# ateme-developers/SVT-AV1-1

Hardware: AMD Instinct MI355X
Metric: 64x64 SAD-search blocks/sec (higher is better)
Workload: dtype u8; 1 GPU; configs[1]: 64x64 full-pel SAD hierarchical ME (centre check + HME L0/L1/L2 + 64x64-area full-pel search of 85 square PUs), 1080p 8-bit, one reference list

## Files before the change

svt-av1-1_amd/csrc/me_hme_impl.h:

```cpp
#pragma once


typedef const __attribute__((address_space(1))) uint32_t gmem_u32;
struct __attribute__((packed, aligned(1))) gmem_u32x4 { uint32_t v[4]; };

__device__ __forceinline__ uint32_t ldu32(const uint8_t* p)
{
    const uintptr_t a = reinterpret_cast<uintptr_t>(p);
    gmem_u32* q = (gmem_u32*)(a & ~(uintptr_t)3);
    const uint32_t sh = (uint32_t)(a & 3u);
    const uint32_t lo = q[0];
    const uint32_t hi = sh ? q[1] : 0u;
    return __builtin_amdgcn_alignbyte(hi, lo, sh);
}

__device__ __forceinline__ uint32_t ldu32_nb(const uint8_t* p)
{
    const uintptr_t a = reinterpret_cast<uintptr_t>(p);
    gmem_u32* q = (gmem_u32*)(a & ~(uintptr_t)3);
    return __builtin_amdgcn_alignbyte(q[1], q[0], (uint32_t)(a & 3u));
}

__device__ __forceinline__ uint32_t wave_sum_u32(uint32_t v)
{
#pragma unroll
    for (int m = 1; m < 64; m <<= 1) v += __shfl_xor(v, m);
    return v;
}

#ifdef SVTHIP_HME_NO_PRIO
#define HME_PRIO(p) do { } while (0)
#else
#define HME_PRIO(p) __builtin_amdgcn_s_setprio(p)
#endif
#ifdef SVTHIP_HME_STAMPS
__device__ unsigned long long g_hme_stamps[8192 * 4 * 8];
#define HME_STAMP(i)                                                                                                          \
    do {                                                                                                                      \
        if (lane == 0 && sbi < 8192u) g_hme_stamps[((size_t)sbi * 4 + (threadIdx.x >> 6)) * 8 + (i)] = __builtin_amdgcn_s_memtime(); \
    } while (0)
__device__ unsigned long long g_hme_loop_phase[2 * 4];
#define HME_LOOP_T(var) const unsigned long long var = __builtin_amdgcn_s_memtime()
#define HME_LOOP_ADD(slot, t1, t0)                                                                                \
    do {                                                                                                          \
        if (lane == 0) atomicAdd(&g_hme_loop_phase[(W == 64 ? 4 : 0) + (slot)], (unsigned long long)((t1) - (t0))); \
    } while (0)
#else
#define HME_STAMP(i) do { } while (0)
#define HME_LOOP_T(var) do { } while (0)
#define HME_LOOP_ADD(slot, t1, t0) do { } while (0)
#endif

constexpr int kHmeLdsPerWave = 7 * 1024;

__device__ __forceinline__ void load_ref_block64(const uint8_t* ref, uint32_t ref_stride, int lane, uint32_t (&tv)[8])
{
    const uint32_t c = (uint32_t)lane & 15u, r0 = (uint32_t)lane >> 4;
    const uint8_t* rp = ref + (size_t)r0 * ref_stride + 4u * c;
#pragma unroll
    for (int k = 0; k < 8; k++) tv[k] = ldu32_nb(rp + (size_t)(4 * k) * ref_stride);
}

__device__ __forceinline__ uint32_t sad_ref_block64(const uint32_t (&tv)[8], const uint32_t* src_lds, int lane)
{
    const uint32_t c = (uint32_t)lane & 15u, r0 = (uint32_t)lane >> 4;
    uint32_t acc4 = 0;
#pragma unroll
    for (int k = 0; k < 8; k++) acc4 = __builtin_amdgcn_sad_u8(src_lds[(r0 + 4 * k) * 16 + c], tv[k], acc4);
    return wave_sum_u32(acc4);
}

__device__ uint32_t wave_block_sad(const uint8_t* src, uint32_t src_stride, const uint8_t* ref, uint32_t ref_stride,
                                   uint32_t H, uint32_t W, int lane, const uint32_t* src_lds = nullptr)
{
    if (src_lds && W == 64 && H == 32) {
        uint32_t tv[8];
        load_ref_block64(ref, ref_stride, lane, tv);
        return sad_ref_block64(tv, src_lds, lane);
    }
    if (W == 64 && (H & 3u) == 0) {
        const uint32_t c = (uint32_t)lane & 15u, r0 = (uint32_t)lane >> 4;
        const uint8_t* sp = src + (size_t)r0 * src_stride + 4u * c;
        const uint8_t* rp = ref + (size_t)r0 * ref_stride + 4u * c;
        uint32_t acc4 = 0;
        for (uint32_t r = 0; r < H; r += 16) {
            uint32_t sv[4], tv[4];
#pragma unroll
            for (int k = 0; k < 4; k++) {
                const bool in = r + 4u * (uint32_t)k < H;
                sv[k] = in ? *reinterpret_cast<const uint32_t*>(sp + (size_t)(4 * k) * src_stride) : 0u;
                tv[k] = in ? ldu32_nb(rp + (size_t)(4 * k) * ref_stride) : 0u;
            }
#pragma unroll
            for (int k = 0; k < 4; k++) acc4 = __builtin_amdgcn_sad_u8(sv[k], tv[k], acc4);
            sp += (size_t)16 * src_stride;
            rp += (size_t)16 * ref_stride;
        }
        return wave_sum_u32(acc4);
    }
    const uint32_t ndw = (W + 3) >> 2;
    const uint32_t n = H * ndw;
    uint32_t acc = 0;
    for (uint32_t i = lane; i < n; i += 64) {
        const uint32_t r = i / ndw, c = i - r * ndw;
        uint32_t s = ldu32(src + (size_t)r * src_stride + 4 * c);
        uint32_t t = ldu32(ref + (size_t)r * ref_stride + 4 * c);
        const uint32_t rem = W - 4 * c;
        if (rem < 4) {
            const uint32_t m = (1u << (8 * rem)) - 1u;
            s &= m;
            t &= m;
        }
        acc = __builtin_amdgcn_sad_u8(s, t, acc);
    }
    return wave_sum_u32(acc);
}

__device__ void wave_sad_loop_generic(const uint8_t* src, uint32_t src_stride, const uint8_t* ref, uint32_t ref_stride,
                                      uint32_t H, uint32_t W, uint32_t ref_stride_raw, int sw, int sh, int lane,
                                      uint32_t* best_sad, int* bx, int* by)
{
    const int npos = sw * sh;
    unsigned long long best = ~0ull;
    const uint32_t ndw = (W + 3) >> 2;
    const uint32_t tail = W & 3u;
    const uint32_t tailmask = tail ? ((1u << (8 * tail)) - 1u) : 0xffffffffu;
#pragma unroll 1
    for (int pos = lane; pos < npos; pos += 64) {
        const int y = pos / sw, x = pos - y * sw;
        const uint8_t* r0 = ref + (size_t)y * ref_stride_raw + x;
        uint32_t acc = 0;
#pragma unroll 1
        for (uint32_t r = 0; r < H; r++) {
            const uint8_t* sp = src + (size_t)r * src_stride;
            const uint8_t* rp = r0 + (size_t)r * ref_stride;
#pragma unroll 2
            for (uint32_t c = 0; c < ndw; c++) {
                uint32_t s = ldu32(sp + 4 * c);
                uint32_t t = ldu32(rp + 4 * c);
                if (c == ndw - 1) {
                    s &= tailmask;
                    t &= tailmask;
                }
                acc = __builtin_amdgcn_sad_u8(s, t, acc);
            }
        }
        const unsigned long long key = ((unsigned long long)acc << 32) | (uint32_t)pos;
        best = key < best ? key : best;
    }
    best = wave_min_u64(best);
    const uint32_t pos = (uint32_t)__builtin_amdgcn_readfirstlane((int)(uint32_t)best);
    *best_sad = (uint32_t)__builtin_amdgcn_readfirstlane((int)(uint32_t)(best >> 32));
    *by = (int)(pos / (uint32_t)sw);
    *bx = (int)(pos - (uint32_t)(*by) * (uint32_t)sw);
}

__device__ __forceinline__ void stage_window_rows(const uint8_t* base, uint32_t ref_stride_raw, int wrows, int pitch, uint32_t* win,
                                                  int lane)
{
    constexpr int NP = 6;
    const int lpr = (pitch + 3) >> 2;
    const int rpp = lpr < 64 ? 64 / lpr : 1;
    const int g = (int)(((uint32_t)lane * ((1u << 16) / (uint32_t)lpr + 1u)) >> 16), q4 = 4 * (lane - g * lpr);
    const bool lane_ok = g < rpp;
    const uintptr_t a0 = reinterpret_cast<uintptr_t>(base) + 4u * (uint32_t)q4;
    for (int r0 = g; r0 < wrows; r0 += NP * rpp) {
        gmem_u32x4 w[NP];
#pragma unroll
        for (int u = 0; u < NP; u++) {
            const int r = min(r0 + u * rpp, wrows - 1);
            const __attribute__((address_space(1))) gmem_u32x4* q = (const __attribute__((address_space(1))) gmem_u32x4*)(a0 + (size_t)r * ref_stride_raw);
#pragma unroll
            for (int k = 0; k < 4; k++) w[u].v[k] = q->v[k];
        }
#pragma unroll
        for (int u = 0; u < NP; u++) {
            const int r = r0 + u * rpp;
            if (lane_ok && r < wrows) {
                uint32_t* o = win + r * pitch + q4;
#pragma unroll
                for (int k = 0; k < 4; k++)
                    if (q4 + k < pitch) o[k] = w[u].v[k];
            }
        }
    }
}

template <int W, bool KEY32 = false>
__device__ void wave_sad_loop_lds(const uint8_t* src, uint32_t src_stride, const uint8_t* ref, uint32_t ref_stride_raw,
                                  int H, int sw, int sh, int lane, uint8_t* lds, int lds_bytes, uint32_t* best_sad,
                                  int* bx, int* by, const uint32_t* shared_src = nullptr)
{
    constexpr int WD = W / 4;
    constexpr int FLUSH = (W == 16) ? 16 : (W == 32 ? 8 : 4);
    const int own_src = shared_src ? 0 : H * WD;
    const uint32_t* srcbuf = shared_src ? shared_src : reinterpret_cast<const uint32_t*>(lds);
    const int noct = (sw + 7) >> 3;
    const int pitch = 2 * noct + WD + 1;
    uint32_t* win = reinterpret_cast<uint32_t*>(lds) + own_src;
    const int avail_rows = (lds_bytes / 4 - own_src) / pitch;
    int band = avail_rows - (2 * H - 2);
    if (band > sh) band = sh;
    if (band < 1) {
        wave_sad_loop_generic(src, src_stride, ref, ref_stride_raw * 2, (uint32_t)H, (uint32_t)W, ref_stride_raw, sw, sh, lane,
                              best_sad, bx, by);
        return;
    }

    for (int i0 = 0; !shared_src && i0 < H * WD; i0 += 256) {
        uint32_t v[4];
#pragma unroll
        for (int k = 0; k < 4; k++) {
            const int i = min(i0 + k * 64 + lane, H * WD - 1);
            const int r = i / WD, c = i - r * WD;
            v[k] = ldu32_nb(src + (uint32_t)r * src_stride + 4u * (uint32_t)c);
        }
#pragma unroll
        for (int k = 0; k < 4; k++) reinterpret_cast<uint32_t*>(lds)[min(i0 + k * 64 + lane, H * WD - 1)] = v[k];
    }

    const int items_row = noct;
    unsigned long long best = ~0ull;
    uint32_t best32 = 0xffffffffu;

    for (int y0 = 0; y0 < sh; y0 += band) {
        const int bh = min(band, sh - y0);
        const int wrows = bh + 2 * H - 2;
        HME_LOOP_T(t_a);
        HME_PRIO(3);
        stage_window_rows(ref + (size_t)y0 * ref_stride_raw, ref_stride_raw, wrows, pitch, win, lane);
        __builtin_amdgcn_wave_barrier();
        asm volatile("s_waitcnt vmcnt(0) lgkmcnt(0)" ::: "memory");
        HME_PRIO(0);
        HME_LOOP_T(t_b);
        HME_LOOP_ADD(0, t_b, t_a);

        const int nitems = items_row * bh;
        int RP = 1, rp_shift = 0;
        while (RP < 8 && nitems * RP * 2 <= 64 && RP * 2 <= H) { RP <<= 1; rp_shift++; }
        const int ipw = 64 >> rp_shift;
        const int part = lane & (RP - 1);
        const uint32_t inv_items = (1u << 20) / (uint32_t)items_row + 1u;
        for (int it0 = 0; it0 < nitems; it0 += ipw) {
            const int item = it0 + (lane >> rp_shift);
            const bool valid = item < nitems;
            const int iy = valid ? (int)(((uint32_t)item * inv_items) >> 20) : 0;
            const int io = valid ? item - iy * items_row : 0;
            uint32_t sad[8];
#pragma unroll
            for (int j = 0; j < 8; j++) sad[j] = 0;
            uint64_t acc0 = 0, acc1 = 0;
            int since = 0;
            for (int r = part; r < H; r += RP) {
                const uint32_t* wr = win + (iy + 2 * r) * pitch + 2 * io;
                const uint32_t* sr = srcbuf + r * WD;
                uint32_t d[WD + 2];
#pragma unroll
                for (int c = 0; c < WD + 2; c++) d[c] = wr[c];
#pragma unroll
                for (int c = 0; c < WD; c++) {
                    const uint32_t sv = sr[c];
                    acc0 = __builtin_amdgcn_qsad_pk_u16_u8(pack64(d[c], d[c + 1]), sv, acc0);
                    acc1 = __builtin_amdgcn_qsad_pk_u16_u8(pack64(d[c + 1], d[c + 2]), sv, acc1);
                }
                if (++since == FLUSH) {
                    since = 0;
                    sad[0] += (uint32_t)acc0 & 0xffffu; sad[1] += ((uint32_t)acc0) >> 16;
                    sad[2] += (uint32_t)(acc0 >> 32) & 0xffffu; sad[3] += (uint32_t)(acc0 >> 48);
                    sad[4] += (uint32_t)acc1 & 0xffffu; sad[5] += ((uint32_t)acc1) >> 16;
                    sad[6] += (uint32_t)(acc1 >> 32) & 0xffffu; sad[7] += (uint32_t)(acc1 >> 48);
                    acc0 = acc1 = 0;
                }
            }
            sad[0] += (uint32_t)acc0 & 0xffffu; sad[1] += ((uint32_t)acc0) >> 16;
            sad[2] += (uint32_t)(acc0 >> 32) & 0xffffu; sad[3] += (uint32_t)(acc0 >> 48);
            sad[4] += (uint32_t)acc1 & 0xffffu; sad[5] += ((uint32_t)acc1) >> 16;
            sad[6] += (uint32_t)(acc1 >> 32) & 0xffffu; sad[7] += (uint32_t)(acc1 >> 48);
            for (int m = 1; m < RP; m <<= 1) {
#pragma unroll
                for (int j = 0; j < 8; j++) sad[j] += __shfl_xor(sad[j], m);
            }
            if (valid && part == 0) {
                const int ys = y0 + iy;
#pragma unroll
                for (int j = 0; j < 8; j++) {
                    const int xs = 8 * io + j;
                    if (xs < sw) {
                        if (KEY32) {
                            best32 = min(best32, (sad[j] << 12) | (uint32_t)(ys * sw + xs));
                        } else {
                            const unsigned long long key = ((unsigned long long)sad[j] << 32) | (uint32_t)(ys * sw + xs);
                            best = key < best ? key : best;
                        }
                    }
                }
            }
        }
        __builtin_amdgcn_wave_barrier();
        HME_LOOP_T(t_c);
        HME_LOOP_ADD(1, t_c, t_b);
    }
    HME_LOOP_T(t_d);
    if (KEY32) {
#pragma unroll
        for (int m = 1; m < 64; m <<= 1) best32 = min(best32, (uint32_t)__shfl_xor((int)best32, m));
        best = ((unsigned long long)(best32 >> 12) << 32) | (best32 & 0xfffu);
    } else {
        best = wave_min_u64(best);
    }
    const uint32_t pos = (uint32_t)__builtin_amdgcn_readfirstlane((int)(uint32_t)best);
    *best_sad = (uint32_t)__builtin_amdgcn_readfirstlane((int)(uint32_t)(best >> 32));
    *by = (int)(pos / (uint32_t)sw);
    *bx = (int)(pos - (uint32_t)(*by) * (uint32_t)sw);
    HME_LOOP_T(t_e);
    HME_LOOP_ADD(2, t_e, t_d);
    HME_LOOP_ADD(3, 1ull, 0ull);
}

template <int W, int H, int SW, int SH>
__device__ void wave_sad_loop_fixed(const uint8_t* ref, uint32_t ref_stride_raw, int lane, uint8_t* lds, const uint32_t* srcbuf,
                                    uint32_t* best_sad, int* bx, int* by)
{
    constexpr int WD = W / 4;
    constexpr int NQ = SW / 4;
    constexpr int RP = 64 / SH;
    constexpr int ROWS = H / RP;
    constexpr int ND = WD + NQ;
    constexpr int PITCH = (ND + 3) & ~3;
    constexpr int WROWS = SH + 2 * H - 2;
    static_assert(RP * SH == 64 && ROWS * RP == H && (RP & (RP - 1)) == 0 && RP >= 2 && RP <= 8, "one wave pass, RP a power of two");
    static_assert(ROWS * W * 255 < 65536 && H * W * 255 < (1 << 20) && SW * SH <= 4096 && (SW & (SW - 1)) == 0, "u16 sums, 32-bit keys");
    static_assert(WROWS * PITCH * 4 <= kHmeLdsPerWave, "the window fits the slice");
    typedef __attribute__((address_space(3))) uint32_t lds_u32;
    typedef uint32_t u32x4_t __attribute__((ext_vector_type(4)));
    typedef uint32_t u32x2_t __attribute__((ext_vector_type(2)));

    uint32_t* win = reinterpret_cast<uint32_t*>(lds);
    HME_PRIO(3);
    stage_window_rows(ref, ref_stride_raw, WROWS, PITCH, win, lane);
    __builtin_amdgcn_wave_barrier();
    asm volatile("s_waitcnt vmcnt(0) lgkmcnt(0)" ::: "memory");
    HME_PRIO(0);

    const int iy = lane / RP, part = lane & (RP - 1);
    const uint32_t* w0 = win + (iy + 2 * part) * PITCH;
    uint64_t acc[NQ];
#pragma unroll
    for (int g = 0; g < NQ; g++) acc[g] = 0;
#pragma unroll
    for (int i = 0; i < ROWS; i++) {
        const int r = part + RP * i;
        const uint32_t* wr = w0 + 2 * RP * i * PITCH;
        lds_u32* wo = (lds_u32*)wr;
        asm("" : "+v"(wo));
        uint32_t d[PITCH];
#pragma unroll
        for (int k = 0; k < PITCH / 4; k++) {
            if (4 * k + 2 >= ND) {
                u32x2_t v = *reinterpret_cast<const u32x2_t*>(wr + 4 * k);
                asm("" : "+v"(v));
                d[4 * k] = v.x; d[4 * k + 1] = v.y; d[4 * k + 2] = d[4 * k + 3] = 0;
            } else {
                u32x4_t v = *reinterpret_cast<const u32x4_t*>(wr + 4 * k);
                asm("" : "+v"(v));
                d[4 * k] = v.x; d[4 * k + 1] = v.y; d[4 * k + 2] = v.z; d[4 * k + 3] = v.w;
            }
        }
        uint64_t odd[ND / 2];
#pragma unroll
        for (int k = 1; k + 1 < ND; k += 2) odd[k / 2] = pack64(wo[k], wo[k + 1]);
        uint32_t sv[WD];
#pragma unroll
        for (int k = 0; k < WD / 4; k++) {
            const uint4 v = *reinterpret_cast<const uint4*>(srcbuf + r * WD + 4 * k);
            sv[4 * k] = v.x; sv[4 * k + 1] = v.y; sv[4 * k + 2] = v.z; sv[4 * k + 3] = v.w;
        }
#pragma unroll
        for (int c = 0; c < WD; c++)
#pragma unroll
            for (int g = 0; g < NQ; g++) {
                const int k = c + g;
                acc[g] = __builtin_amdgcn_qsad_pk_u16_u8((k & 1) ? odd[k / 2] : pack64(d[k], d[k + 1]), sv[c], acc[g]);
            }
    }
    __builtin_amdgcn_wave_barrier();

    uint32_t key = 0xffffffffu;
#pragma unroll
    for (int g = 0; g < NQ; g++) {
        uint32_t v[4] = {(uint32_t)acc[g] & 0xffffu, (uint32_t)acc[g] >> 16, (uint32_t)(acc[g] >> 32) & 0xffffu, (uint32_t)(acc[g] >> 48)};
#pragma unroll
        for (int j = 0; j < 4; j++) {
            v[j] += dpp_fetch<0xB1>(v[j]);
            v[j] += dpp_fetch<0x4E>(v[j]);
            if (RP == 8) v[j] += dpp_fetch<0x141>(v[j]);
        }
        key = min3u((v[0] << 12) | (uint32_t)(4 * g), (v[1] << 12) | (uint32_t)(4 * g + 1), key);
        key = min3u((v[2] << 12) | (uint32_t)(4 * g + 2), (v[3] << 12) | (uint32_t)(4 * g + 3), key);
    }
    key |= (uint32_t)(iy * SW);
    key = min(key, dpp_fetch<0xB1>(key));
    key = min(key, dpp_fetch<0x4E>(key));
    key = min(key, dpp_fetch<0x124>(key));
    key = min(key, dpp_fetch<0x128>(key));
    const uint32_t best = min(min((uint32_t)__builtin_amdgcn_readlane((int)key, 0), (uint32_t)__builtin_amdgcn_readlane((int)key, 16)),
                              min((uint32_t)__builtin_amdgcn_readlane((int)key, 32), (uint32_t)__builtin_amdgcn_readlane((int)key, 48)));
    const uint32_t pos = best & 0xfffu;
    *best_sad = best >> 12;
    *by = (int)(pos / (uint32_t)SW);
    *bx = (int)(pos % (uint32_t)SW);
}

__device__ void wave_sad_loop_l0(const uint8_t* src, uint32_t src_stride, const uint8_t* ref, uint32_t ref_stride_raw, int sw, int sh,
                                 int lane, uint8_t* lds, int lds_bytes, uint32_t* best_sad, int* bx, int* by,
                                 const uint32_t* shared_src = nullptr)
{
    constexpr int H = 8, WD = 4;
    const int own_src = shared_src ? 0 : H * WD;
    const uint32_t* srcbuf = shared_src ? shared_src : reinterpret_cast<const uint32_t*>(lds);
    const int nit = (sw + 15) >> 4;
    const int pitch = 4 * nit + 4;
    uint32_t* win = reinterpret_cast<uint32_t*>(lds) + own_src;
    const int avail_rows = (lds_bytes / 4 - own_src) / pitch;
    int band = avail_rows - (2 * H - 2);
    if (band > sh) band = sh;
    if (band < 1 || sw * sh > 65536) {
        wave_sad_loop_lds<16>(src, src_stride, ref, ref_stride_raw, H, sw, sh, lane, lds, lds_bytes, best_sad, bx, by, shared_src);
        return;
    }
    if (!shared_src && lane < H * WD)
        reinterpret_cast<uint32_t*>(lds)[lane] = ldu32_nb(src + (uint32_t)(lane >> 2) * src_stride + 4u * (uint32_t)(lane & 3));
    uint32_t best = 0xffffffffu;
    const uint32_t inv_nit = (1u << 20) / (uint32_t)nit + 1u;
    for (int y0 = 0; y0 < sh; y0 += band) {
        const int bh = min(band, sh - y0);
        HME_PRIO(3);
        stage_window_rows(ref + (size_t)y0 * ref_stride_raw, ref_stride_raw, bh + 2 * H - 2, pitch, win, lane);
        __builtin_amdgcn_wave_barrier();
        asm volatile("s_waitcnt vmcnt(0) lgkmcnt(0)" ::: "memory");
        HME_PRIO(0);
        const int nitems = nit * bh;
        auto track = [&](const uint64_t* acc, int iy, int io, bool valid) {
            const int xs0 = 16 * io;
            const uint32_t base = (uint32_t)((y0 + iy) * sw + xs0);
            if ((sw & 15) == 0) {
                uint32_t lb = 0xffffffffu;
#pragma unroll
                for (int g = 0; g < 4; g++) {
                    const uint32_t lo = (uint32_t)acc[g], hi = (uint32_t)(acc[g] >> 32), ix = base + 4u * (uint32_t)g;
                    lb = min3u((lo << 16) | ix, (lo & 0xffff0000u) | (ix + 1u), lb);
                    lb = min3u((hi << 16) | (ix + 2u), (hi & 0xffff0000u) | (ix + 3u), lb);
                }
                best = min(best, valid ? lb : 0xffffffffu);
                return;
            }
#pragma unroll
            for (int g = 0; g < 4; g++) {
                const uint32_t lo = (uint32_t)acc[g], hi = (uint32_t)(acc[g] >> 32);
                const uint32_t sad4[4] = {lo << 16, lo & 0xffff0000u, hi << 16, hi & 0xffff0000u};
#pragma unroll
                for (int j = 0; j < 4; j++) {
                    const int xs = xs0 + 4 * g + j;
                    const uint32_t key = (valid && xs < sw) ? (sad4[j] + base + (uint32_t)(4 * g + j)) : 0xffffffffu;
                    best = min(best, key);
                }
            }
        };
        auto row_sads = [&](const uint32_t* wr, int r, uint64_t* acc) {
            const uint4 da = *reinterpret_cast<const uint4*>(wr);
            const uint4 db = *reinterpret_cast<const uint4*>(wr + 4);
            const uint4 sv = *reinterpret_cast<const uint4*>(srcbuf + r * WD);
            const uint32_t d[8] = {da.x, da.y, da.z, da.w, db.x, db.y, db.z, db.w};
            const uint32_t s4[4] = {sv.x, sv.y, sv.z, sv.w};
#pragma unroll
            for (int c = 0; c < WD; c++)
#pragma unroll
                for (int g = 0; g < 4; g++)
                    acc[g] = __builtin_amdgcn_qsad_pk_u16_u8(pack64(d[c + g], d[c + g + 1]), s4[c], acc[g]);
        };
        int it0 = 0;
        for (; nitems - it0 >= 57; it0 += 64) {
            const int item = min(it0 + lane, nitems - 1);
            const bool valid = it0 + lane < nitems;
            const int iy = (int)(((uint32_t)item * inv_nit) >> 20), io = item - iy * nit;
            const uint32_t* w0 = win + iy * pitch + 4 * io;
            uint64_t acc[4] = {0, 0, 0, 0};
#pragma unroll
            for (int r = 0; r < H; r++) row_sads(w0 + 2 * r * pitch, r, acc);
            track(acc, iy, io, valid);
        }
        while (it0 < nitems) {
            const int rem = nitems - it0;
            const int rp_shift = rem > 32 ? 1 : rem > 16 ? 1 : rem > 8 ? 2 : 3;
            const int RP = 1 << rp_shift, take = min(rem, 64 >> rp_shift);
            const int slot = lane >> rp_shift, part = lane & (RP - 1);
            const int item = it0 + min(slot, take - 1);
            const int iy = (int)(((uint32_t)item * inv_nit) >> 20), io = item - iy * nit;
            const uint32_t* w0 = win + iy * pitch + 4 * io;
            uint64_t acc[4] = {0, 0, 0, 0};
            for (int r = part; r < H; r += RP) row_sads(w0 + 2 * r * pitch, r, acc);
            for (int m = 1; m < RP; m <<= 1) {
#pragma unroll
                for (int g = 0; g < 4; g++) {
                    const uint32_t lo = (uint32_t)acc[g] + (uint32_t)__shfl_xor((int)(uint32_t)acc[g], m);
                    const uint32_t hi = (uint32_t)(acc[g] >> 32) + (uint32_t)__shfl_xor((int)(uint32_t)(acc[g] >> 32), m);
                    acc[g] = pack64(lo, hi);
                }
            }
            track(acc, iy, io, slot < take && part == 0);
            it0 += take;
        }
        __builtin_amdgcn_wave_barrier();
    }
#pragma unroll
    for (int m = 1; m < 64; m <<= 1) best = min(best, (uint32_t)__shfl_xor((int)best, m));
    best = (uint32_t)__builtin_amdgcn_readfirstlane((int)best);
    const uint32_t pos = best & 0xffffu;
    *best_sad = best >> 16;
    *by = (int)(pos / (uint32_t)sw);
    *bx = (int)(pos - (uint32_t)(*by) * (uint32_t)sw);
}

__device__ __forceinline__ void clamp_center(int& x, int& y, int ox, int oy, int pw, int ph)
{
    x = (ox + x < -63) ? (-63 - ox) : x;
    x = (ox + x > pw - 1) ? (x - ((ox + x) - (pw - 1))) : x;
    y = (oy + y < -63) ? (-63 - oy) : y;
    y = (oy + y > ph - 1) ? (y - ((oy + y) - (ph - 1))) : y;
}

__device__ __forceinline__ void clip_window(int& xo, int& yo, int& sw, int& sh, int ox, int oy, int padw, int padh,
                                            int pw, int ph)
{
    xo = (ox + xo < -padw) ? (-padw - ox) : xo;
    sw = (ox + xo < -padw) ? (sw - (-padw - (ox + xo))) : sw;
    xo = (ox + xo > pw - 1) ? (xo - ((ox + xo) - (pw - 1))) : xo;
    sw = (ox + xo + sw > pw) ? max(1, sw - ((ox + xo + sw) - pw)) : sw;
    yo = (oy + yo < -padh) ? (-padh - oy) : yo;
    sh = (oy + yo < -padh) ? (sh - (-padh - (oy + yo))) : sh;
    yo = (oy + yo > ph - 1) ? (yo - ((oy + yo) - (ph - 1))) : yo;
    sh = (oy + yo + sh > ph) ? max(1, sh - ((oy + yo + sh) - ph)) : sh;
}

__device__ __forceinline__ int s16(int v) { return (int)(int16_t)v; }

__device__ __forceinline__ int round_hme_width(int w)
{
    return (w < 8) ? 8 : ((w & 7) ? (w + (w - ((w >> 3) << 3))) : w);
}

struct HmeShared {
    unsigned long long cost[8];
    int rx[3][4], ry[3][4];
    unsigned long long rs[3][4];
    int cx, cy;
    unsigned long long hcost;
    svthip_fullpel_desc desc;
    __attribute__((aligned(16))) uint32_t src2[32 * 16];
    __attribute__((aligned(16))) uint32_t src1[16 * 8];
    __attribute__((aligned(16))) uint32_t src0[8 * 4];
};


__device__ __forceinline__ void hme_center_sb(const uint8_t* __restrict__ pool, const svthip_pa_picture& cur, const svthip_pa_picture& ref,
                                              const svthip_me_params& P, uint32_t list_index, int ox, int oy, uint32_t sbi,
                                              const uint32_t* __restrict__ l0_best_mv64, uint32_t l0_mv_stride,
                                              svthip_fullpel_desc* __restrict__ out_desc, int16_t* __restrict__ out_center,
                                              int16_t* __restrict__ hme_state, HmeShared& sh, uint8_t* hme_lds)
{
    const int tid = threadIdx.x, lane = tid & 63;
    const int wave = __builtin_amdgcn_readfirstlane(tid >> 6);
    uint8_t* wlds = hme_lds + wave * kHmeLdsPerWave;
    const int pw = cur.width, ph = cur.height;
    const uint32_t sb_w = (uint32_t)min(64, pw - ox), sb_h = (uint32_t)min(64, ph - oy);
    const int nw = P.number_hme_search_region_in_width, nh = P.number_hme_search_region_in_height;

    const uint8_t* cur_full = pool + cur.full_offset + (size_t)68 * cur.full_stride + 68;
    const uint8_t* ref_full = pool + ref.full_offset + (size_t)68 * ref.full_stride + 68;
    const uint8_t* src = cur_full + (size_t)oy * cur.full_stride + ox;
    HME_STAMP(0);
    HME_PRIO(3);

    const bool center_path = (P.temporal_layer_index > 0) || (list_index == 0);
    const int tw = P.hme_level0_total_search_area_width, th = P.hme_level0_total_search_area_height;
    const bool full_sb = sb_w == 64 && sb_h == 64;
    uint32_t cand_tv[8];
    if (full_sb && center_path) {
        int x = wave == 1 ? tw : 0, y = wave == 2 ? -th : (wave == 3 ? th : 0);
        clamp_center(x, y, ox, oy, ref.width, ref.height);
        load_ref_block64(ref_full + (size_t)(oy + y) * ref.full_stride + ox + x, ref.full_stride * 2, lane, cand_tv);
    }
    if (full_sb) {
#pragma unroll
        for (int k = 0; k < 2; k++) {
            const int i = tid + 256 * k;
            sh.src2[i] = *reinterpret_cast<const uint32_t*>(src + (size_t)(i >> 4) * (cur.full_stride * 2) + 4 * (i & 15));
        }
        if (tid < 128) {
            const uint8_t* s1 = pool + cur.quarter_offset + (size_t)(32 + (oy >> 1)) * cur.quarter_stride + 32 + (ox >> 1);
            sh.src1[tid] = ldu32_nb(s1 + (size_t)(tid >> 3) * (cur.quarter_stride * 2) + 4 * (tid & 7));
        } else if (tid < 160) {
            const int i = tid - 128;
            const uint8_t* s0 = pool + cur.sixteenth_offset + (size_t)(16 + (oy >> 2)) * cur.sixteenth_stride + 16 + (ox >> 2);
            sh.src0[i] = ldu32_nb(s0 + (size_t)(i >> 2) * (cur.sixteenth_stride * 2) + 4 * (i & 3));
        }
        __syncthreads();
    }
    const uint32_t* src2_lds = full_sb ? sh.src2 : nullptr;
    HME_STAMP(1);

    const uint32_t mv64 = (list_index == 1 && l0_best_mv64) ? l0_best_mv64[(size_t)sbi * l0_mv_stride] : 0u;
    const int dx = s16(0 - (s16((int)(mv64 & 0xffffu)) >> 2));
    const int dy = s16(0 - (s16((int)(mv64 >> 16)) >> 2));

    if (tid == 0 && hme_state && list_index == 0) hme_state[25 * (size_t)sbi + 24] = 0;
    int xc = 0, yc = 0;
    unsigned long long hme_cost = ~0ull;
    if (center_path) {
        const int ncand = (list_index == 1) ? 5 : 4;
        const int cxs[5] = {0, tw, 0, 0, dx}, cys[5] = {0, 0, -th, th, dy};
        for (int c = wave; c < ncand; c += 4) {
            uint32_t sad;
            if (full_sb && c == wave) {
                sad = sad_ref_block64(cand_tv, src2_lds, lane);
            } else {
                int x = cxs[c], y = cys[c];
                clamp_center(x, y, ox, oy, ref.width, ref.height);
                sad = wave_block_sad(src, cur.full_stride * 2, ref_full + (size_t)(oy + y) * ref.full_stride + ox + x, ref.full_stride * 2,
                                     sb_h >> 1, sb_w, lane, src2_lds);
            }
            if (lane == 0) sh.cost[c] = (unsigned long long)(sad << 1) << 8;
        }
        __syncthreads();
        {
            const unsigned long long zero = sh.cost[0], b = sh.cost[1], c = sh.cost[2], d = sh.cost[3];
            const unsigned long long dir = (list_index == 1) ? sh.cost[4] : 0xFFFFFFFFFFFFFull;
            unsigned long long best = zero;
            best = b < best ? b : best;
            best = c < best ? c : best;
            best = d < best ? d : best;
            best = dir < best ? dir : best;
            if (best == zero) { xc = 0; yc = 0; }
            else if (best == b) { xc = tw; yc = 0; }
            else if (best == c) { xc = 0; yc = s16(0 - th); }
            else if (best == dir) { xc = dx; yc = dy; }
            else { xc = 0; yc = th; }
        }

        if (P.enable_hme_flag && sb_h == 64) {
            const int nreg = nw * nh;
            const int16_t* st = hme_state ? hme_state + 25 * (size_t)sbi : nullptr;
            const bool carried = st && list_index == 1 && st[24];
            if (wave < nreg) {
                const int rw = wave % nw, rh = wave / nw;
                const int k = rw * 2 + rh;
                int x0 = xc, y0 = yc, x1 = xc, y1 = yc, x2 = xc, y2 = yc;
                if (carried) { x0 = st[k]; y0 = st[4 + k]; x1 = st[8 + k]; y1 = st[12 + k]; x2 = st[16 + k]; y2 = st[20 + k]; }
                uint32_t sad0 = 0, sad1 = 0, sad2 = 0;
                HME_STAMP(2);
                if (P.enable_hme_level0_flag) {
                    const uint32_t mx = P.hme_level0_multiplier_x, my = P.hme_level0_multiplier_y;
                    int sw = s16((int)((P.hme_level0_search_area_in_width_array[rw] * mx) / 100));
                    int shh = s16((int)((P.hme_level0_search_area_in_height_array[rh] * my) / 100));
                    int xd = s16(xc >> 2), yd = s16(yc >> 2);
                    for (int j = rw; j > 0;) { j--; xd = s16(xd + s16((int)((P.hme_level0_search_area_in_width_array[j] * mx) / 100))); }
                    for (int j = rh; j > 0;) { j--; yd = s16(yd + s16((int)((P.hme_level0_search_area_in_height_array[j] * my) / 100))); }
                    int xo = s16(-s16((int)(((tw * mx) / 100) >> 1)) + xd);
                    int yo = s16(-s16((int)(((th * my) / 100) >> 1)) + yd);
                    const int o_x = ox >> 2, o_y = oy >> 2;
                    clip_window(xo, yo, sw, shh, o_x, o_y, 15, 15, ref.width >> 2, ref.height >> 2);
                    const uint8_t* s = pool + cur.sixteenth_offset + (size_t)(16 + o_y) * cur.sixteenth_stride + 16 + o_x;
                    const uint8_t* r = pool + ref.sixteenth_offset + (size_t)(16 + o_y + yo) * ref.sixteenth_stride + 16 + o_x + xo;
                    int bx, by;
                    if (sb_w == 64)
                        wave_sad_loop_l0(s, cur.sixteenth_stride * 2, r, ref.sixteenth_stride, sw, shh, lane, wlds, kHmeLdsPerWave, &sad0,
                                         &bx, &by, sh.src0);
                    else
                        wave_sad_loop_generic(s, cur.sixteenth_stride * 2, r, ref.sixteenth_stride * 2, (sb_h >> 2) >> 1, sb_w >> 2,
                                              ref.sixteenth_stride, sw, shh, lane, &sad0, &bx, &by);
                    x0 = s16(s16(bx + xo) * 4);
                    y0 = s16(s16(by + yo) * 4);
                }
                HME_STAMP(3);
                if (P.enable_hme_level1_flag) {
                    int sw = round_hme_width((int)(int16_t)P.hme_level1_search_area_in_width_array[rw]);
                    int shh = (int)(int16_t)P.hme_level1_search_area_in_height_array[rh];
                    int xo = s16(-(sw >> 1) + (x0 >> 1)), yo = s16(-(shh >> 1) + (y0 >> 1));
                    const int o_x = ox >> 1, o_y = oy >> 1;
                    clip_window(xo, yo, sw, shh, o_x, o_y, 31, 31, ref.width >> 1, ref.height >> 1);
                    const uint8_t* s = pool + cur.quarter_offset + (size_t)(32 + o_y) * cur.quarter_stride + 32 + o_x;
                    const uint8_t* r = pool + ref.quarter_offset + (size_t)(32 + o_y + yo) * ref.quarter_stride + 32 + o_x + xo;
                    int bx, by;
                    if (sb_w == 64 && sw == 16 && shh == 16)
                        wave_sad_loop_fixed<32, 16, 16, 16>(r, ref.quarter_stride, lane, wlds, sh.src1, &sad1, &bx, &by);
                    else if (sb_w == 64 && sw * shh <= 4096)
                        wave_sad_loop_lds<32, true>(s, cur.quarter_stride * 2, r, ref.quarter_stride, 16, sw, shh, lane, wlds,
                                                    kHmeLdsPerWave, &sad1, &bx, &by, sh.src1);
                    else if (sb_w == 64)
                        wave_sad_loop_lds<32>(s, cur.quarter_stride * 2, r, ref.quarter_stride, 16, sw, shh, lane, wlds,
                                              kHmeLdsPerWave, &sad1, &bx, &by, sh.src1);
                    else
                        wave_sad_loop_generic(s, cur.quarter_stride * 2, r, ref.quarter_stride * 2, (sb_h >> 1) >> 1, sb_w >> 1,
                                              ref.quarter_stride, sw, shh, lane, &sad1, &bx, &by);
                    x1 = s16(s16(bx + xo) * 2);
                    y1 = s16(s16(by + yo) * 2);
                }
                HME_STAMP(4);
                if (P.enable_hme_level2_flag) {
                    int sw = round_hme_width((int)(int16_t)P.hme_level2_search_area_in_width_array[rw]);
                    int shh = (int)(int16_t)P.hme_level2_search_area_in_height_array[rh];
                    int xo = s16(-(sw >> 1) + x1), yo = s16(-(shh >> 1) + y1);
                    clip_window(xo, yo, sw, shh, ox, oy, 63, 63, ref.width, ref.height);
                    const uint8_t* r = ref_full + (size_t)(oy + yo) * ref.full_stride + ox + xo;
                    int bx, by;
                    if (sb_w == 64 && sw == 8 && shh == 8)
                        wave_sad_loop_fixed<64, 32, 8, 8>(r, ref.full_stride, lane, wlds, sh.src2, &sad2, &bx, &by);
                    else if (sb_w == 64 && sw * shh <= 4096)
                        wave_sad_loop_lds<64, true>(src, cur.full_stride * 2, r, ref.full_stride, 32, sw, shh, lane, wlds,
                                                    kHmeLdsPerWave, &sad2, &bx, &by, sh.src2);
                    else if (sb_w == 64)
                        wave_sad_loop_lds<64>(src, cur.full_stride * 2, r, ref.full_stride, 32, sw, shh, lane, wlds,
                                              kHmeLdsPerWave, &sad2, &bx, &by, sh.src2);
                    else
                        wave_sad_loop_generic(src, cur.full_stride * 2, r, ref.full_stride * 2, sb_h >> 1, sb_w, ref.full_stride, sw,
                                              shh, lane, &sad2, &bx, &by);
                    x2 = s16(bx + xo);
                    y2 = s16(by + yo);
                }
                HME_STAMP(5);
                if (lane == 0) {
                    sh.rx[0][k] = x0; sh.ry[0][k] = y0; sh.rs[0][k] = (unsigned long long)sad0 * 2;
                    sh.rx[1][k] = x1; sh.ry[1][k] = y1; sh.rs[1][k] = (unsigned long long)sad1 * 2;
                    sh.rx[2][k] = x2; sh.ry[2][k] = y2; sh.rs[2][k] = (unsigned long long)sad2 * 2;
                }
            }
            __syncthreads();
            if (tid == 0) {
                int lvl = -1;
                if (P.enable_hme_level0_flag && !P.enable_hme_level1_flag && !P.enable_hme_level2_flag) lvl = 0;
                if (P.enable_hme_level1_flag && !P.enable_hme_level2_flag) lvl = 1;
                if (P.enable_hme_level2_flag) lvl = 2;
                int xh = 0, yh = 0;
                unsigned long long bs = ~0ull;
                if (lvl >= 0) {
                    xh = sh.rx[lvl][0]; yh = sh.ry[lvl][0];
                    bs = sh.rs[lvl][0];
                    int w = 1, h = 0;
                    while (h < nh) {
                        while (w < nw) {
                            const int k = w * 2 + h;
                            if (sh.rs[lvl][k] < bs) { xh = sh.rx[lvl][k]; yh = sh.ry[lvl][k]; bs = sh.rs[lvl][k]; }
                            w++;
                        }
                        w = 0;
                        h++;
                    }
                }
                unsigned long long hcost = lvl == 2 ? bs << 8 : ~0ull;
                if (P.enable_hme_level2_flag) {
                    const int total = nh * nw;
                    if (P.ref_poc_equal && list_index == 1 && total > 1) {
                        uint32_t from = 0xE4u;
                        for (int q = 0; q < total - 1; q++)
                            for (int n = q + 1; n < total; n++) {
                                const int a = (q / nw) * 2 + (q % nw), b = (n / nw) * 2 + (n % nw);
                                if (sh.rs[2][a] > sh.rs[2][b]) {
                                    const int tx = sh.rx[2][a], ty = sh.ry[2][a];
                                    const uint32_t fa = (from >> (2 * a)) & 3u, fb = (from >> (2 * b)) & 3u;
                                    const unsigned long long ts = sh.rs[2][a];
                                    sh.rx[2][a] = sh.rx[2][b]; sh.ry[2][a] = sh.ry[2][b]; sh.rs[2][a] = sh.rs[2][b];
                                    sh.rx[2][b] = tx; sh.ry[2][b] = ty; sh.rs[2][b] = ts;
                                    from ^= ((fa ^ fb) << (2 * a)) | ((fa ^ fb) << (2 * b));
                                }
                            }
                        xh = sh.rx[2][1];
                        yh = sh.ry[2][1];
                        const uint32_t f1 = (from >> 2) & 3u;
                        const bool live = (int)(f1 >> 1) < nw && (int)(f1 & 1u) < nh;
                        hcost = live ? sh.rs[2][1] << 8 : ~0ull;
                    }
                }
                sh.cx = xh;
                sh.cy = yh;
                sh.hcost = hcost;
                if (hme_state) {
                    int16_t* so = hme_state + 25 * (size_t)sbi;
                    for (int k = 0; k < 4; k++) {
                        const bool live = ((k >> 1) < nw) && ((k & 1) < nh);
                        for (int l = 0; l < 3; l++) {
                            so[8 * l + k] = (int16_t)(live ? sh.rx[l][k] : (carried ? so[8 * l + k] : 0));
                            so[8 * l + 4 + k] = (int16_t)(live ? sh.ry[l][k] : (carried ? so[8 * l + 4 + k] : 0));
                        }
                    }
                    so[24] = 1;
                }
            }
            __syncthreads();
            xc = sh.cx;
            yc = sh.cy;
            hme_cost = sh.hcost;
        }
    }

    HME_PRIO(3);
    if ((xc != 0 || yc != 0) && P.is_used_as_reference_flag) {
        clamp_center(xc, yc, ox, oy, ref.width, ref.height);
        unsigned long long z, hcost;
        if (hme_cost != ~0ull && ox < ref.width && oy < ref.height) {
            z = sh.cost[0];
            hcost = hme_cost;
        } else {
            __syncthreads();
            if (wave < 2) {
                const int x = wave ? xc : 0, y = wave ? yc : 0;
                const uint32_t sad = wave_block_sad(src, cur.full_stride * 2, ref_full + (size_t)(oy + y) * ref.full_stride + ox + x,
                                                    ref.full_stride * 2, sb_h >> 1, sb_w, lane, src2_lds);
                if (lane == 0) sh.cost[6 + wave] = (unsigned long long)(sad << 1) << 8;
            }
            __syncthreads();
            z = sh.cost[6];
            hcost = sh.cost[7];
        }
        const unsigned long long m = z < hcost ? z : hcost;
        if (m == z) { xc = 0; yc = 0; }
    }

    HME_STAMP(6);
    if (tid == 0) {
        int sw = min((int)P.search_area_width, 127), shh = min((int)P.search_area_height, 127);
        int xo = s16(xc - (sw >> 1)), yo = s16(yc - (shh >> 1));
        clip_window(xo, yo, sw, shh, ox, oy, 63, 63, pw, ph);
        svthip_fullpel_desc d;
        d.src_offset = (int32_t)(cur.full_offset + (int64_t)(68 + oy) * cur.full_stride + 68 + ox);
        d.ref_offset = (int32_t)(ref.full_offset + (int64_t)(68 + oy + yo) * ref.full_stride + 68 + ox + xo);
        d.x_search_area_origin = xo;
        d.y_search_area_origin = yo;
        d.search_area_width = sw;
        d.search_area_height = shh;
        out_desc[sbi] = d;
        sh.desc = d;
        if (out_center) {
            out_center[2 * sbi] = (int16_t)xc;
            out_center[2 * sbi + 1] = (int16_t)yc;
        }
    }
}
```

Baseline: 9.930 million blocks/s.

## Add single-band L0 SAD fast path and aligned quad-load window staging

Adds a specialised L0 HME search path for the case where the source block is shared, the search width is a multiple of 16 and the whole window fits in one LDS band. It iterates items with incremental row/column tracking and handles the tail by splitting rows across lanes with shuffle reductions. It also adds a QUAD variant of window staging that uses precomputed offsets and 16-byte LDS stores, applied to the fixed-size search as well. The intent is to cut address arithmetic, per-band loop overhead and tracking cost, at the price of extra code paths and more register pressure.

```diff
diff --git a/svt-av1-1_amd/csrc/me_hme_impl.h b/svt-av1-1_amd/csrc/me_hme_impl.h
--- a/svt-av1-1_amd/csrc/me_hme_impl.h
+++ b/svt-av1-1_amd/csrc/me_hme_impl.h
@@ -155,9 +155,42 @@
     *bx = (int)(pos - (uint32_t)(*by) * (uint32_t)sw);
 }
 
+template <bool QUAD = false>
 __device__ __forceinline__ void stage_window_rows(const uint8_t* base, uint32_t ref_stride_raw, int wrows, int pitch, uint32_t* win,
                                                   int lane)
 {
+    if constexpr (QUAD) {
+        constexpr int NP = 6;
+        typedef uint32_t u32x4_t __attribute__((ext_vector_type(4)));
+        typedef const __attribute__((address_space(1))) uint8_t gmem_u8;
+        const int lpr = pitch >> 2;
+        const int rpp = lpr < 64 ? 64 / lpr : 1;
+        const int g = (int)(((uint32_t)lane * ((1u << 16) / (uint32_t)lpr + 1u)) >> 16), q4 = 4 * (lane - g * lpr);
+        const bool lane_ok = g < rpp;
+        gmem_u8* b = (gmem_u8*)base;
+        const uint32_t step = (uint32_t)rpp * ref_stride_raw;
+        const uint32_t last = (uint32_t)(wrows - 1) * ref_stride_raw + 4u * (uint32_t)q4;
+        uint32_t off = (uint32_t)g * ref_stride_raw + 4u * (uint32_t)q4;
+        uint32_t* o = win + g * pitch + q4;
+        for (int r0 = g; r0 < wrows; r0 += NP * rpp) {
+            gmem_u32x4 w[NP];
+#pragma unroll
+            for (int u = 0; u < NP; u++) {
+                const __attribute__((address_space(1))) gmem_u32x4* q =
+                    (const __attribute__((address_space(1))) gmem_u32x4*)(b + min(off + (uint32_t)u * step, last));
+#pragma unroll
+                for (int k = 0; k < 4; k++) w[u].v[k] = q->v[k];
+            }
+            asm volatile("" ::: "memory");
+#pragma unroll
+            for (int u = 0; u < NP; u++)
+                if (lane_ok && r0 < wrows - u * rpp)
+                    *reinterpret_cast<u32x4_t*>(o + u * rpp * pitch) = u32x4_t{w[u].v[0], w[u].v[1], w[u].v[2], w[u].v[3]};
+            off += NP * step;
+            o += NP * rpp * pitch;
+        }
+        return;
+    }
     constexpr int NP = 6;
     const int lpr = (pitch + 3) >> 2;
     const int rpp = lpr < 64 ? 64 / lpr : 1;
@@ -337,7 +370,7 @@
 
     uint32_t* win = reinterpret_cast<uint32_t*>(lds);
     HME_PRIO(3);
-    stage_window_rows(ref, ref_stride_raw, WROWS, PITCH, win, lane);
+    stage_window_rows<true>(ref, ref_stride_raw, WROWS, PITCH, win, lane);
     __builtin_amdgcn_wave_barrier();
     asm volatile("s_waitcnt vmcnt(0) lgkmcnt(0)" ::: "memory");
     HME_PRIO(0);
@@ -411,6 +444,96 @@
     *bx = (int)(pos % (uint32_t)SW);
 }
 
+__device__ __forceinline__ void l0_row_sads(const uint32_t* wr, const uint32_t* sr, uint64_t* acc)
+{
+    typedef uint32_t u32x4_t __attribute__((ext_vector_type(4)));
+    const u32x4_t da = *reinterpret_cast<const u32x4_t*>(wr);
+    const u32x4_t db = *reinterpret_cast<const u32x4_t*>(wr + 4);
+    const uint4 sv = *reinterpret_cast<const uint4*>(sr);
+    const uint32_t d[8] = {da.x, da.y, da.z, da.w, db.x, db.y, db.z, db.w};
+    const uint32_t s4[4] = {sv.x, sv.y, sv.z, sv.w};
+#pragma unroll
+    for (int c = 0; c < 4; c++)
+#pragma unroll
+        for (int g = 0; g < 4; g++) acc[g] = __builtin_amdgcn_qsad_pk_u16_u8(pack64(d[c + g], d[c + g + 1]), s4[c], acc[g]);
+}
+
+__device__ __forceinline__ uint32_t l0_item_min(const uint64_t* acc)
+{
+    uint32_t lb = 0xffffffffu;
+#pragma unroll
+    for (int g = 0; g < 4; g++) {
+        const uint32_t lo = (uint32_t)acc[g], hi = (uint32_t)(acc[g] >> 32);
+        lb = min3u((lo << 16) | (uint32_t)(4 * g), (lo & 0xffff0000u) | (uint32_t)(4 * g + 1), lb);
+        lb = min3u((hi << 16) | (uint32_t)(4 * g + 2), (hi & 0xffff0000u) | (uint32_t)(4 * g + 3), lb);
+    }
+    return lb;
+}
+
+__device__ void wave_sad_loop_l0_oneband(const uint8_t* ref, uint32_t ref_stride_raw, int nit, int sh, int lane, uint8_t* lds,
+                                         const uint32_t* srcbuf, uint32_t* best_sad, int* bx, int* by)
+{
+    constexpr int H = 8, WD = 4;
+    const int pitch = 4 * nit + 4;
+    const uint32_t* win = reinterpret_cast<const uint32_t*>(lds);
+    HME_PRIO(3);
+    stage_window_rows<true>(ref, ref_stride_raw, sh + 2 * H - 2, pitch, reinterpret_cast<uint32_t*>(lds), lane);
+    __builtin_amdgcn_wave_barrier();
+    asm volatile("s_waitcnt vmcnt(0) lgkmcnt(0)" ::: "memory");
+    HME_PRIO(0);
+
+    const int nitems = nit * sh;
+    const uint32_t inv_nit = (1u << 20) / (uint32_t)nit + 1u;
+    const uint32_t qs = (64u * inv_nit) >> 20, rs = 64u - qs * (uint32_t)nit;
+    uint32_t best = 0xffffffffu;
+    uint32_t item = (uint32_t)lane;
+    uint32_t iy = (item * inv_nit) >> 20, io = item - iy * (uint32_t)nit;
+    int it0 = 0;
+    for (; nitems - it0 >= 57; it0 += 64) {
+        const bool valid = item < (uint32_t)nitems;
+        const uint32_t* w0 = win + (valid ? 4u * (item + iy) : 0u);
+        uint64_t acc[4] = {0, 0, 0, 0};
+#pragma unroll
+        for (int r = 0; r < H; r++) l0_row_sads(w0 + 2 * r * pitch, srcbuf + r * WD, acc);
+        const uint32_t key = l0_item_min(acc) + 16u * item;
+        best = min(best, valid ? key : 0xffffffffu);
+        item += 64;
+        io += rs;
+        const bool carry = io >= (uint32_t)nit;
+        io -= carry ? (uint32_t)nit : 0u;
+        iy += qs + (carry ? 1u : 0u);
+    }
+    while (it0 < nitems) {
+        const int rem = nitems - it0;
+        const int rp_shift = rem > 16 ? 1 : rem > 8 ? 2 : 3;
+        const int RP = 1 << rp_shift, take = min(rem, 64 >> rp_shift);
+        const int slot = lane >> rp_shift, part = lane & (RP - 1);
+        const uint32_t ri = (uint32_t)(it0 + min(slot, take - 1));
+        const uint32_t* w0 = win + 4u * (ri + ((ri * inv_nit) >> 20));
+        uint64_t acc[4] = {0, 0, 0, 0};
+        for (int r = part; r < H; r += RP) l0_row_sads(w0 + 2 * r * pitch, srcbuf + r * WD, acc);
+        for (int m = 1; m < RP; m <<= 1) {
+#pragma unroll
+            for (int g = 0; g < 4; g++) {
+                const uint32_t lo = (uint32_t)acc[g] + (uint32_t)__shfl_xor((int)(uint32_t)acc[g], m);
+                const uint32_t hi = (uint32_t)(acc[g] >> 32) + (uint32_t)__shfl_xor((int)(uint32_t)(acc[g] >> 32), m);
+                acc[g] = pack64(lo, hi);
+            }
+        }
+        const uint32_t key = l0_item_min(acc) + 16u * ri;
+        best = min(best, (slot < take && part == 0) ? key : 0xffffffffu);
+        it0 += take;
+    }
+    __builtin_amdgcn_wave_barrier();
+#pragma unroll
+    for (int m = 1; m < 64; m <<= 1) best = min(best, (uint32_t)__shfl_xor((int)best, m));
+    best = (uint32_t)__builtin_amdgcn_readfirstlane((int)best);
+    const uint32_t pos = best & 0xffffu, sw = 16u * (uint32_t)nit;
+    *best_sad = best >> 16;
+    *by = (int)(pos / sw);
+    *bx = (int)(pos - (uint32_t)(*by) * sw);
+}
+
 __device__ void wave_sad_loop_l0(const uint8_t* src, uint32_t src_stride, const uint8_t* ref, uint32_t ref_stride_raw, int sw, int sh,
                                  int lane, uint8_t* lds, int lds_bytes, uint32_t* best_sad, int* bx, int* by,
                                  const uint32_t* shared_src = nullptr)
@@ -426,6 +549,10 @@
     if (band > sh) band = sh;
     if (band < 1 || sw * sh > 65536) {
         wave_sad_loop_lds<16>(src, src_stride, ref, ref_stride_raw, H, sw, sh, lane, lds, lds_bytes, best_sad, bx, by, shared_src);
+        return;
+    }
+    if (shared_src && (sw & 15) == 0 && band == sh) {
+        wave_sad_loop_l0_oneband(ref, ref_stride_raw, nit, sh, lane, lds, shared_src, best_sad, bx, by);
         return;
     }
     if (!shared_src && lane < H * WD)
```

Measured after the change: 10.06 million blocks/s (median of 6 runs). +1.3%, better.
